# Equim-chan/Mortal

Measured on NVIDIA H100. Metric: table-steps/sec batched self-play, higher is better.
Workload: dtype u8/i32 env + bf16 policy net

## Files before the change

### mortal_b200/csrc/mjx_kernels.cu

```cuda
#include <cstdint>
#include <cstdio>
#include <cstring>
#include <initializer_list>
#include <mutex>
#include <string>
#include <vector>

#include "../../include/mjx.h"
#include "mjx_sp.cuh"
#include "mjx_policy.cuh"
#include "mjx_replay.cuh"
#include "mjx_validate.cuh"
#include "mjx_mjai.cuh"
#include "mjx_mjai_write.cuh"
#include "mjx_stat.cuh"
#include "mjx_grp.cuh"
#include "mjx_reward.cuh"
#include "mjx_invisible.cuh"
#include "mjx_state.cuh"
#include "mjx_nn.cuh"
#include "mjx_tables_host.h"

using namespace mjx;

// ... 424 lines not shown
    recompute_dora_factor(c);

__global__ void k_state_init(TableState* tabs, int n, const u8* player_ids) {
    const int t = blockIdx.x * blockDim.x + threadIdx.x;
    if (t < n) { tabs[t].viewer1 = (u8)(player_ids[t] + 1); tabs[t].gflags = GF_ALIVE; tabs[t].last_kawa_tile = T_NONE;
                 for (int s = 0; s < 4; s++) tabs[t].priv[s].last_self_tsumo = T_NONE; }
}

__global__ void __launch_bounds__(STEP_WARPS * 32) k_state_update(EnvView V, Tables T, const u64* __restrict__ words,
                                                                    const u64* __restrict__ payload, u32* __restrict__ cans) {
    STATE_KERNEL_PROLOGUE
    const u64 w = words[i];
    const int p = c.S->viewer1 - 1;
    if (w != 0) {
        apply_event(c, w, payload ? payload + (size_t)i * REPLAY_KYOKU_WORDS : nullptr, false);
        __syncwarp();
        for (int q = lane; q < NV; q += 32) reinterpret_cast<uint4*>(g)[q] = dst[q];
    }
    if (lane == 0) cans[i] = (u32)c.S->priv[p].cans | ((u32)c.S->priv[p].target_actor << 16);
}

__global__ void __launch_bounds__(STEP_WARPS * 32) k_state_view(EnvView V, Tables T, int index, mjx_player_view* out) {
    STATE_KERNEL_PROLOGUE
    if (i != index) return;
    if (lane == 0) state_view(c, c.S->viewer1 - 1, out);
}

__global__ void __launch_bounds__(STEP_WARPS * 32) k_state_rows(EnvView V, Tables T, const u8* __restrict__ at_kan_select) {
    STATE_KERNEL_PROLOGUE
    const int p = c.S->viewer1 - 1;
    const bool kan = at_kan_select && at_kan_select[i];
    const u16 cans_bits = c.S->priv[p].cans;
    const u64 discards = (cans_bits & CAN_DISCARD) ? discard_candidates(c, p) : 0;
    write_mask_row(c, V, i, legal_mask(c, p, kan, discards));
    if (lane == 0) { V.row_table[i] = i; V.row_seat[i] = (u8)(p | (kan ? 4 : 0)); V.row_step[i] = 0; if (i == 0) *V.n_rows = V.n_tables; }
}

__global__ void __launch_bounds__(STEP_WARPS * 32) k_state_query(EnvView V, Tables T, int index, int what, const i32* __restrict__ args,
                                                                   i32* __restrict__ out) {
    STATE_KERNEL_PROLOGUE
    if (i != index) return;
    const int p = c.S->viewer1 - 1;
    if (what == 0) {
        u8 ura[5];
        const int n_ura = min(max(args[1], 0), 5);
        for (int k = 0; k < n_ura; k++) ura[k] = (u8)args[2 + k];
        bool ok;
        const Point pt = agari_points_ura(c, p, args[0] != 0, ura, n_ura, &ok);
        if (lane == 0) { out[0] = pt.ron; out[1] = pt.tsumo_ko; out[2] = pt.tsumo_oya; out[3] = ok ? 1 : 0; }
    } else if (what == 1) {
        const bool r = rule_based_agari(c, p);
        if (lane == 0) out[0] = r ? 1 : 0;
    } else if (what == 2) {
        const u64 m = discard_candidates(c, p);
        if (lane == 0) { out[0] = (i32)(u32)m; out[1] = (i32)(u32)(m >> 32); }
    } else if (what == 3) {
        EncCtx e; e.S = c.S; e.T = T; e.bm = nullptr; e.sv = nullptr; e.seat = p; e.kan_select = false; e.lane = lane;
        e.dora_factor = c.df; e.parts = 0;
        const u64 m = unconditional_tenpai_discards(e, c);
        if (lane == 0) { out[0] = (i32)(u32)m; out[1] = (i32)(u32)(m >> 32); }
    } else if (what == 4) {
        Reaction r;
        i32 err = 0;
        const bool okd = decode_action(c.S, p, args[0], args[1], r, &err);
        if (lane == 0) {
            u64 w = 0;
            if (okd) {
                const int ty = r.type == R_DAHAI ? LOG_DAHAI : r.type == R_CHI ? LOG_CHI : r.type == R_PON ? LOG_PON :
                               r.type == R_DAIMINKAN ? LOG_DAIMINKAN : r.type == R_KAKAN ? LOG_KAKAN : r.type == R_ANKAN ? LOG_ANKAN :
                               r.type == R_REACH ? LOG_REACH : r.type == R_HORA ? LOG_HORA : r.type == R_RYUKYOKU ? LOG_RYUKYOKU : 0;
                w = log_word(ty, r.actor, r.target, r.pai, r.tsumogiri, 0, r.consumed[0], r.consumed[1], r.consumed[2], r.consumed[3], 0);
            }
            out[0] = (i32)(u32)w; out[1] = (i32)(u32)(w >> 32); out[2] = okd ? 0 : (err ? err : ERR_ILLEGAL_ACTION);
        }
    }
}

constexpr int SP_WARPS = 4;
constexpr int MJX_HOST_COPY_GROUPS = 4;
constexpr int MJX_SP_MAX_LANES = 4;

__global__ void k_sp_begin(SpGlobal G) {
    if (threadIdx.x < SP_SLOTS) G.wl_count[threadIdx.x] = 0;
    if (threadIdx.x == 0) {
        if (G.counters[2]) G.counters[3] += 1;
        G.counters[0] = 0; G.counters[1] = 0; G.counters[2] = 0; G.counters[4] = 0; G.counters[5] = 0;
    }
}

#define SP_ROW_PROLOGUE                                                                         \
    __shared__ u8 s_df[SP_WARPS][40];                                                           \
    const int warp = threadIdx.x >> 5, lane = threadIdx.x & 31;                                 \
    const int gwarp = blockIdx.x * SP_WARPS + warp, nwarps = gridDim.x * SP_WARPS;              \
    SpCtx s; s.G = G; s.T = T; s.df = s_df[warp]; s.lane = lane;

#define SP_ROW_RANGE                                                                            \
    const int span_ = max(min(*V.n_rows, row_hi) - row_lo, 0);                                  \
    const int r0 = row_lo + (int)((long long)span_ * part / parts), r1 = row_lo + (int)((long long)span_ * (part + 1) / parts);

__global__ void __launch_bounds__(SP_WARPS * 32) k_sp_init(SpGlobal G, Tables T, EnvView V, int row_lo, int row_hi, int part, int parts) {
    SP_ROW_PROLOGUE
    SP_ROW_RANGE
    for (int row = r0 + gwarp; row < r1; row += nwarps)
        sp_stage_init(s, V.tables + V.row_table[row], row, V.row_table[row], V.row_seat[row] & 3);
}

template <int KIND>
__global__ void __launch_bounds__(SP_THREADS) k_sp_expand(SpGlobal G, Tables T, int level) {
    __shared__ SpExpandBatch sb;
    SpBlk B; B.tid = threadIdx.x; B.nthr = blockDim.x; B.bid = blockIdx.x; B.nblk = gridDim.x;
    sp_expand_level<KIND>(G, T, sb, B, level);
}

template <int KIND>
__global__ void __launch_bounds__(SP_THREADS) k_sp_eval(SpGlobal G, int level) {
    SpBlk B; B.tid = threadIdx.x; B.nthr = blockDim.x; B.bid = blockIdx.x; B.nblk = gridDim.x;
    if (KIND == 0) {
        __shared__ SpEvalDBatch sd;
        sp_eval_d_level(G, sd, B, level);
    } else {
        __shared__ SpEvalWBatch sw[SP_THREADS / 32];
        sp_eval_w_level<KIND == 2>(G, sw, B, level);
    }
}

__global__ void k_sp_tables(float* p_tab) {
    const int i = blockIdx.x * blockDim.x + threadIdx.x;
    if (i < SP_NTS_DIM * SP_NTS_DIM) sp_fill_ptab_block(p_tab + (size_t)i * 4 * SP_TRI, i / SP_NTS_DIM, i % SP_NTS_DIM);
}

__global__ void k_sp_mark(SpGlobal G, int which) { G.counters[4 + which] = min(G.counters[1], G.edge_cap); }

__global__ void __launch_bounds__(256) k_sp_densify(SpGlobal G) {
    SpBlk B; B.tid = threadIdx.x; B.nthr = blockDim.x; B.bid = blockIdx.x; B.nblk = gridDim.x;
    sp_densify(G, B);
}

__global__ void __launch_bounds__(128) k_sp_score(SpGlobal G, Tables T) {
    const int b = G.counters[4], e_end = G.counters[5];
    for (int e = b + blockIdx.x * blockDim.x + threadIdx.x; e < e_end; e += gridDim.x * blockDim.x) sp_score_edge(G, T, e);
}

__global__ void __launch_bounds__(SP_WARPS * 32) k_sp_finalize(SpGlobal G, Tables T, EnvView V, float* __restrict__ obs, int row_lo,
                                                               int row_hi, int part, int parts) {
    SP_ROW_PROLOGUE
    SP_ROW_RANGE
    for (int row = r0 + gwarp; row < r1; row += nwarps)
        sp_stage_finalize(s, row, obs + (size_t)row * OBS_ROWS_V4 * OBS_COLS);
}

__global__ void __launch_bounds__(256) k_sp_release(SpGlobal G) {
    SpBlk B; B.tid = threadIdx.x; B.nthr = blockDim.x; B.bid = blockIdx.x; B.nblk = gridDim.x;
    sp_release(G, B);
}

__global__ void k_policy_test(EnvView V, int kind, i64* actions, i64* trace, float* q_out) {
    const int n_rows = *V.n_rows;
    for (int r = blockIdx.x * blockDim.x + threadIdx.x; r < n_rows; r += gridDim.x * blockDim.x) {
        const int t = V.row_table[r], seat = V.row_seat[r] & 3, kan = (V.row_seat[r] >> 2) & 1;
        u64 m = 0;
        for (int i = 0; i < ACTION_SPACE; i++) if (V.masks[(size_t)r * ACTION_SPACE + i]) m |= 1ull << i;
        const TableState* S = V.tables + t;
        const SeatPrivate& P = S->priv[seat];
        u64 h = policy_hash(S->nonce, S->key, (u64)t, V.row_step[r], (u32)seat, (u32)kan);
        int a = test_policy(kind, h, kan != 0, m, P.keep_shanten, P.next_shanten);
        actions[r] = a;
// ... 84 lines not shown

template <typename Tp>
int upload(const std::vector<Tp>& v, const Tp** out) {
    Tp* d = nullptr;
    CU(cudaMalloc(&d, v.size() * sizeof(Tp)));
    CU(cudaMemcpy(d, v.data(), v.size() * sizeof(Tp), cudaMemcpyHostToDevice));
    *out = d;
    return 0;
}

}

struct mjx_env {
    int n_tables = 0, row_cap = 0, obs_version = 4, shuffle_kind = 0, quick_eval = 1;
    bool first = true;
    EnvView V;
    u64 *d_nonces = nullptr, *d_keys = nullptr;
    i64* d_dummy_actions = nullptr;
    u8* d_guard = nullptr;
    u8* d_quick_eval = nullptr;
    SpGlobal sp;
    int sp_enabled = 1, sp_wanted = 1;
    SpGlobal sp_lane[MJX_SP_MAX_LANES - 1];
    int sp_lanes = 1, sp_lanes_alloc = 1;
    int sp_grid_x = 10, sp_grid_e = 16;
    int sp_thr_x = SP_THREADS, sp_thr_e = SP_THREADS;
    long long sp_want_slots = 0;
    cudaStream_t sp_stream[MJX_SP_MAX_LANES] = {};
    cudaEvent_t ev_sp_fork = nullptr, ev_sp_store = nullptr, ev_sp_join[MJX_SP_MAX_LANES] = {};
    unsigned char* d_compact = nullptr;
    cudaEvent_t ev_enc[3] = {nullptr, nullptr, nullptr};
    bool time_encode = false;
    ReplayView R{};
    bool replay = false;
    long long r_n_hdr = 0, r_n_kyoku = 0;
    bool viewpoints = false;
    int* d_enc_work = nullptr;
    EncStoreArgs enc_args{};
    cudaStream_t copy_stream = nullptr;
    cudaEvent_t ev_rows = nullptr, ev_sp = nullptr, ev_grp[MJX_HOST_COPY_GROUPS] = {};
    long long launches = 0;
    bool is_state = false;
    u64 *d_state_words = nullptr, *d_state_pay = nullptr;
    u32* d_state_cans = nullptr;
    unsigned char* d_state_misc = nullptr;
};

static void set_enc_args(mjx_env* env, int version) {
    const ObsLayout L = make_layout(version);
    env->enc_args.rows = L.rows; env->enc_args.bm_rows = L.bm_rows; env->enc_args.n_sv = L.n_sv;
    env->enc_args.compact_bytes = L.bm_rows * 8 + L.n_sv * OBS_COLS * 4;
    env->enc_args.n_slices = (L.rows + OBS_SLICE_ROWS - 1) / OBS_SLICE_ROWS;
    env->enc_args.ver = version;
}

template <int VER>
static void launch_features(mjx_env* env, cudaStream_t st) {
    k_encode_features<VER><<<g_sm_count, EncF<VER>::WARPS * 32, EncF<VER>::SMEM, st>>>(env->V, g_T, env->d_compact, env->d_enc_work);
}

static int sp_alloc(SpGlobal& G, long long want) {
    int hc = 1 << 20;
    while (hc < want && hc < (1 << 26)) hc <<= 1;
    G.hash_cap = hc;
    G.p_tab = g_sp_p_tab;
    G.wl_cap = hc / 2;
    G.edge_cap = hc * 2;
    G.score_cap = hc;
    CU(cudaMalloc(&G.hkey, (size_t)G.hash_cap * sizeof(u64)));
    CU(cudaMalloc(&G.nsig, (size_t)G.hash_cap * sizeof(SpSigP)));
    CU(cudaMalloc(&G.einfo, (size_t)G.hash_cap * sizeof(u64)));
    CU(cudaMalloc(&G.vals, (size_t)G.hash_cap * SP_VALS * sizeof(float)));
    CU(cudaMalloc(&G.sid, (size_t)G.hash_cap * sizeof(u32)));
    CU(cudaMalloc(&G.dkey, (size_t)G.hash_cap * sizeof(u64)));
    CU(cudaMalloc(&G.echild, (size_t)G.edge_cap * sizeof(u32)));
    CU(cudaMalloc(&G.evid, (size_t)G.edge_cap * sizeof(u32)));
    CU(cudaMemset(G.evid, 0, (size_t)G.edge_cap * sizeof(u32)));
    CU(cudaMalloc(&G.emeta, (size_t)G.edge_cap * sizeof(u16)));
    CU(cudaMalloc(&G.eowner, (size_t)G.edge_cap * sizeof(u32)));
    CU(cudaMalloc(&G.leaf_scores, (size_t)G.score_cap * 4 * sizeof(float)));
    CU(cudaMalloc(&G.wl, (size_t)SP_SLOTS * G.wl_cap * sizeof(u32)));
    CU(cudaMalloc(&G.wl_count, SP_SLOTS * sizeof(i32)));
    CU(cudaMalloc(&G.counters, 8 * sizeof(i32)));
    CU(cudaMemset(G.counters, 0, 8 * sizeof(i32)));
    CU(cudaMemset(G.wl_count, 0, SP_SLOTS * sizeof(i32)));
    CU(cudaMemset(G.hkey, 0xFF, (size_t)G.hash_cap * sizeof(u64)));
    return MJX_OK;
}
static SpGlobal& sp_of(mjx_env* env, int lane) { return lane == 0 ? env->sp : env->sp_lane[lane - 1]; }
static void sp_free(SpGlobal& G) {
    cudaFree(G.hkey); cudaFree(G.nsig); cudaFree(G.einfo); cudaFree(G.vals); cudaFree(G.sid); cudaFree(G.dkey); cudaFree(G.echild); cudaFree(G.evid); cudaFree(G.emeta);
    cudaFree(G.eowner); cudaFree(G.leaf_scores); cudaFree(G.wl); cudaFree(G.wl_count); cudaFree(G.counters);
}
static int sp_ensure_lanes(mjx_env* env, int lanes) {
    if (!env->ev_sp_fork) {
        CU(cudaEventCreateWithFlags(&env->ev_sp_fork, cudaEventDisableTiming));
        CU(cudaEventCreateWithFlags(&env->ev_sp_store, cudaEventDisableTiming));
    }
    for (int g = 0; g < lanes; g++)
        if (!env->sp_stream[g]) {
            CU(cudaStreamCreateWithFlags(&env->sp_stream[g], cudaStreamNonBlocking));
            CU(cudaEventCreateWithFlags(&env->ev_sp_join[g], cudaEventDisableTiming));
        }
    for (int g = env->sp_lanes_alloc; g < lanes; g++) {
        SpGlobal& G = env->sp_lane[g - 1];
        memset(&G, 0, sizeof G);
        G.rows = env->sp.rows;
        int rc = sp_alloc(G, env->sp_want_slots * 2 / lanes);
        if (rc) return rc;
        env->sp_lanes_alloc = g + 1;
    }
    return MJX_OK;
}

extern "C" {

const char* mjx_last_error(void) { return g_err.c_str(); }

int mjx_init(const char* data_dir, int device) {
    std::lock_guard<std::mutex> lk(g_mu);
    if (g_ready) {
        if (device != g_device) return fail(MJX_ERR_ARG, "mjx_init: already initialised on another device");
        return MJX_OK;
    }
    int n_dev = 0;
    cudaError_t e = cudaGetDeviceCount(&n_dev);
    if (e != cudaSuccess || n_dev == 0)
        return fail(MJX_ERR_CUDA, "mjx_init: no CUDA device (this library has no CPU path)");
    CU(cudaSetDevice(device));
    cudaDeviceProp prop;
    CU(cudaGetDeviceProperties(&prop, device));
    g_sm_count = prop.multiProcessorCount;
    HostTables H;
    if (!load_host_tables(data_dir, H)) return fail(MJX_ERR_TABLES, "mjx_init: " + H.error);
    int rc;
    if ((rc = upload(H.suhai, &g_T.suhai))) return rc;
    if ((rc = upload(H.jihai, &g_T.jihai))) return rc;
    if ((rc = upload(H.agari_keys, &g_T.agari_keys))) return rc;
    if ((rc = upload(H.agari_divs, &g_T.agari_divs))) return rc;
    if ((rc = upload(H.agari_ndivs, &g_T.agari_ndivs))) return rc;
    CU(cudaFuncSetAttribute(k_encode_features<1>, cudaFuncAttributeMaxDynamicSharedMemorySize, (int)EncF<1>::SMEM));
    CU(cudaFuncSetAttribute(k_encode_features<2>, cudaFuncAttributeMaxDynamicSharedMemorySize, (int)EncF<2>::SMEM));
    CU(cudaFuncSetAttribute(k_encode_features<3>, cudaFuncAttributeMaxDynamicSharedMemorySize, (int)EncF<3>::SMEM));
    CU(cudaFuncSetAttribute(k_encode_features<4>, cudaFuncAttributeMaxDynamicSharedMemorySize, (int)EncF<4>::SMEM));
    {
        short tab[4][OBS_MAX_SV];
        for (int v = 1; v <= 4; v++) {
            const ObsLayout L = make_layout(v);
            for (int i = 0; i < OBS_MAX_SV; i++) tab[v - 1][i] = i < L.n_sv ? L.sv_row[i] : (short)-1;
        }
        CU(cudaMemcpyToSymbol(c_sv_row, tab, sizeof tab));
    }
    CU(cudaFuncSetAttribute(k_encode_store, cudaFuncAttributeMaxDynamicSharedMemorySize, (int)ENCS_SMEM_BYTES));
    {
        float* pt = nullptr;
        CU(cudaMalloc(&pt, sizeof(float) * SP_NTS_DIM * SP_NTS_DIM * 4 * SP_TRI));
        k_sp_tables<<<(SP_NTS_DIM * SP_NTS_DIM + 63) / 64, 64>>>(pt);
        CU(cudaGetLastError());
        CU(cudaDeviceSynchronize());
        g_sp_p_tab = pt;
    }
    g_device = device;
    g_ready = true;
    return MJX_OK;
}

int mjx_obs_rows(int version) {
    switch (version) {
        case 1: return 938;
        case 2: return 942;
        case 3: return 934;
        case 4: return 1012;
        default: return MJX_ERR_ARG;
    }
}
// ... 1134 lines not shown
```

### mortal_b200/csrc/mjx_sp.cuh

```cuda
#pragma once
#include "mjx_obs.cuh"

namespace mjx {

constexpr int SP_T_MAX = 17;
constexpr int SP_SHANTEN_THRES = 3;
constexpr int SP_MAX_TILES_LEFT = 34 * 4 - 1 - 13;
constexpr int SP_SLOTS = 8;
constexpr int SP_B = 32;
constexpr int SP_THREADS = 128;
constexpr int SP_MAX_EDGES = 37;
constexpr u64 SP_EMPTY = ~0ull;
constexpr u32 SP_NO_CHILD = 0xFFFFFFFFu;
constexpr u32 SP_DR_NONE = 0x3FFFFu, SP_DI_NONE = 0xFFFFFFu;
constexpr int SP_VALS = 3 * SP_T_MAX;

#ifdef MJX_HOST_EMUL
#define SP_FMUL(a, b) ((a) * (b))
#define SP_FADD(a, b) ((a) + (b))
#define SP_FDIV(a, b) ((a) / (b))
#define SP_SYNC() ((void)0)
#else
#define SP_FMUL(a, b) __fmul_rn((a), (b))
#define SP_FADD(a, b) __fadd_rn((a), (b))
// ... 48 lines not shown
MJX_HD u32 sp_hash64(u64 x) {
    x ^= x >> 33; x *= 0xff51afd7ed558ccdull; x ^= x >> 33; x *= 0xc4ceb9fe1a85ec53ull; x ^= x >> 33;
    return (u32)x;
}

struct alignas(16) SpSigP { u32 w[4]; };
MJX_D SpSigP sp_sig_pack(const HandSig& h) {
    SpSigP p;
    p.w[0] = h.idx[0] | ((u32)h.kinds << 21); p.w[1] = h.idx[1] | ((u32)h.pairs << 21);
    p.w[2] = h.idx[2] | ((u32)h.kkinds << 21); p.w[3] = h.idx[3] | ((u32)h.kpairs << 21);
    return p;
}
MJX_D HandSig sp_sig_unpack(const SpSigP& p) {
    HandSig h;
    for (int i = 0; i < 4; i++) h.idx[i] = p.w[i] & 0x1FFFFFu;
    h.kinds = (int)(p.w[0] >> 21); h.pairs = (int)(p.w[1] >> 21); h.kkinds = (int)(p.w[2] >> 21); h.kpairs = (int)(p.w[3] >> 21);
    return h;
}

template <bool ADD>
MJX_D int sp_candidate_shanten(const Tables& T, const SpSigP& sg, const u8* others, int t, int c0, int len_div3) {
    const int sx = t / 9, pos = t - 9 * sx;
    const u32 w5 = sx < 3 ? c_pow5[pos] : c_pow5[pos + 2];
    const u32 idx = (sg.w[sx] & 0x1FFFFFu) + (ADD ? w5 : 0u - w5);
    const u64 r = sx < 3 ? ld_row(T.suhai, idx, SUHAI_ROWS) : ld_row(T.jihai, idx, JIHAI_ROWS);
    int v = 1 << 20;
#pragma unroll
    for (int a = 0; a <= 4; a++) {
        if (a <= len_div3) {
            const int b = len_div3 - a;
            v = min(v, (int)others[5 + a] + (int)((r >> (4 * b)) & 0xF));
            v = min(v, (int)others[a] + (int)((r >> (4 * (5 + b))) & 0xF));
        }
    }
    int sh = v - 1;
    if (sh <= 0 || len_div3 < 4) return sh;
    int kinds = (int)(sg.w[0] >> 21), pairs = (int)(sg.w[1] >> 21), kkinds = (int)(sg.w[2] >> 21), kpairs = (int)(sg.w[3] >> 21);
    const bool yao = is_yaokyuu(t);
    if (ADD) { kinds += c0 == 0; pairs += c0 == 1; if (yao) { kkinds += c0 == 0; kpairs += c0 == 1; } }
    else { kinds -= c0 == 1; pairs -= c0 == 2; if (yao) { kkinds -= c0 == 1; kpairs -= c0 == 2; } }
    sh = min(sh, 7 - pairs + max(7 - kinds, 0) - 1);
    if (sh > 0) sh = min(sh, 14 - kkinds - (kpairs > 0 ? 1 : 0) - 1);
    return sh;
}

struct SpRow {
    u8 tehai_len_div3, is_menzen, prefer_riichi, calc_double_riichi, calc_haitei;
    u8 bakaze, jikaze, num_doras_in_fuuro, n_dora;
    u8 dora_ind[5];
    u8 melds[16];
    u8 n_chis, n_pons, n_minkans, n_ankans;
    u8 T;
    u8 n_left;
    u8 avail;
    u8 has_values;
    u8 can_discard;
    u8 cd_flag;
    u8 after_riichi, last_self_tsumo;
    i8 cur_shanten;
    u8 seat;
    i32 table;
    u32 root;
    float fallback_ev;
    SpKey root_key;
};

struct SpGlobal {
    SpRow* rows;
    u64* hkey;
    SpSigP* nsig;
    u64* einfo;
    u64* dkey;
    float* vals;
    u32* sid;
    u32* echild;
    u32* evid;
    u16* emeta;
    u32* eowner;
    float* leaf_scores;
    u32* wl;
    i32* wl_count;
    const float* p_tab;
    i32* counters;
    i32 row_base;
    i32 hash_cap, wl_cap, edge_cap, score_cap;
};

MJX_CONST float c_uradora_prob[5][13] = {
    {0.639485f, 0.327801f, 0.0327134f, 0.f, 0.f, 0.f, 0.f, 0.f, 0.f, 0.f, 0.f, 0.f, 0.f},
    {0.406736f, 0.42281f, 0.147966f, 0.021674f, 0.0008142f, 0.f, 0.f, 0.f, 0.f, 0.f, 0.f, 0.f, 0.f},
    {0.257516f, 0.406819f, 0.246851f, 0.0757724f, 0.0122266f, 0.0008004f, 1.43e-5f, 0.f, 0.f, 0.f, 0.f, 0.f, 0.f},
    {0.162199f, 0.346513f, 0.301539f, 0.142396f, 0.0401276f, 0.0066491f, 0.0005575f, 1.85e-5f, 0.f, 0.f, 0.f, 0.f, 0.f},
    {0.101768f, 0.275319f, 0.313742f, 0.20189f, 0.081774f, 0.0215394f, 0.0035918f, 0.0003607f, 1.52e-5f, 3e-7f, 0.f, 0.f, 0.f},
};
MJX_CONST u8 c_discard_priority[38] = {6, 5, 4, 3, 2, 3, 4, 5, 6, 6, 5, 4, 3, 2, 3, 4, 5, 6, 6, 5, 4, 3, 2, 3, 4, 5, 6,
                                        7, 7, 7, 7, 7, 7, 7, 1, 1, 1, 0};

MJX_D int cmp_discard_priority(int l, int r) {
    int pl = c_discard_priority[l], pr = c_discard_priority[r];
    if (pl != pr) return pl < pr ? -1 : 1;
    if (l != r) return r < l ? -1 : 1;
    return 0;
}

struct SpBlk { int tid, nthr, bid, nblk; };

MJX_HD bool sp_slot_is_w(int slot) { return (slot & 1) != 0; }
MJX_HD int sp_slot_shanten(int slot) { return 3 - (slot >> 1); }
MJX_D float* sp_vals(const SpGlobal& G, u32 vid, int which) { return G.vals + ((size_t)vid * 3 + which) * SP_T_MAX; }
MJX_D u32 sp_einfo_begin(u64 e) { return (u32)e; }
MJX_D int sp_einfo_n(u64 e) { return (int)((e >> 32) & 0xFF); }
MJX_D int sp_einfo_sum(u64 e) { return (int)((e >> 40) & 0xFF); }
MJX_D int sp_einfo_cmask(u64 e) { return (int)((e >> 48) & 0xF); }

MJX_D void sp_set_overflow(const SpGlobal& G) { G.counters[2] = 1; }

constexpr u32 SP_SID_POS = (1u << 28) - 1u;
MJX_D u32 sp_level_base(const SpGlobal& G, int level) {
    u32 b = 0;
    for (int l = 0; l < level; l++) b += (u32)min(G.wl_count[l], G.wl_cap);
    return b;
}
MJX_D u32 sp_vid(const SpGlobal& G, u32 slot) {
    const u32 s = G.sid[slot];
    return sp_level_base(G, (int)(s >> 28)) + (s & SP_SID_POS);
}
MJX_DN void sp_densify(const SpGlobal& G, const SpBlk& B) {
    if (G.counters[2]) return;
    u32 base[SP_SLOTS];
    for (int l = 0; l < SP_SLOTS; l++) base[l] = sp_level_base(G, l);
    const int n = min(G.counters[1], G.edge_cap), leaf_b = G.counters[4], leaf_e = G.counters[5];
    for (int e = B.bid * B.nthr + B.tid; e < n; e += B.nblk * B.nthr) {
        if (e >= leaf_b && e < leaf_e) continue;
        const u32 c = G.echild[e];
        u32 v = SP_NO_CHILD;
        if (c != SP_NO_CHILD) { const u32 sd = G.sid[c]; v = base[sd >> 28] + (sd & SP_SID_POS); }
        G.evid[e] = v;
    }
}

MJX_D void sp_prefetch(const float* p) {
#ifndef MJX_HOST_EMUL
    asm volatile("prefetch.global.L1 [%0];" ::"l"(p));
    asm volatile("prefetch.global.L1 [%0];" ::"l"(p + 32));
#else
    (void)p;
#endif
}
MJX_D i32 sp_atomic_add(i32* p, i32 v) {
#ifdef MJX_HOST_EMUL
    const i32 o = *p; *p += v; return o;
#else
    return atomicAdd(p, v);
#endif
}
MJX_D void sp_atomic_or(u32* p, u32 v) {
#ifdef MJX_HOST_EMUL
    *p |= v;
#else
    atomicOr(p, v);
#endif
}

MJX_DN u32 sp_intern(const SpGlobal& G, u64 key, bool& won) {
    const u32 mask = (u32)G.hash_cap - 1;
    u32 h = sp_hash64(key) & mask;
    won = false;
    for (int probe = 0; probe < 8192; probe++, h = (h + 1) & mask) {
#ifdef MJX_HOST_EMUL
        const u64 cur = G.hkey[h];
        if (cur == key) return h;
        if (cur == SP_EMPTY) { G.hkey[h] = key; won = true; return h; }
#else
        const u64 cur = __ldcg(reinterpret_cast<const unsigned long long*>(G.hkey + h));
        if (cur == key) return h;
        if (cur == SP_EMPTY) {
            const u64 prev = atomicCAS(reinterpret_cast<unsigned long long*>(G.hkey + h), (unsigned long long)SP_EMPTY,
                                       (unsigned long long)key);
            if (prev == SP_EMPTY) { won = true; return h; }
            if (prev == key) return h;
        }
#endif
    }
    sp_set_overflow(G);
    return SP_NO_CHILD;
}

struct SpExpandBatch {
    u64 key[SP_B];
    u32 slot[SP_B];
    SpSigP sig[SP_B];
    u8 akas[SP_B], len[SP_B];
    u8 teh[SP_B][34], wall[SP_B][34];
    u8 oth[SP_B][4][12];
    u32 cand[SP_B][2], eff[SP_B][2];
    u8 split[SP_B], ne[SP_B], sumreq[SP_B], cmask[SP_B];
    u16 cand_off[SP_B + 1], e_off[SP_B + 1];
    u16 cand_list[SP_B * 34];
    u32 edge[SP_B * SP_MAX_EDGES];
    u32 win[SP_B * SP_MAX_EDGES];
    i32 n_cand, n_edge, e_base, n_win, w_base;
};

MJX_D u64 sp_mask64(const u32* m) { return (u64)m[0] | ((u64)m[1] << 32); }

template <int KIND>
MJX_DN void sp_expand_batch(const SpGlobal& G, const Tables& T, SpExpandBatch& S, const SpBlk& B, int level, int first, int nb) {
    constexpr bool IS_W = KIND != 0, LEAF = KIND == 2;
    const int k = sp_slot_shanten(level);
    const u32* list = G.wl + (size_t)level * G.wl_cap;
    SP_PFOR(st, nb) {
        const u32 slot = list[first + st];
        const u64 key = G.hkey[slot];
        const SpRow& R = G.rows[sp_key_row(key)];
        S.slot[st] = slot; S.key[st] = key;
        S.sig[st] = G.nsig[slot];
        S.akas[st] = (u8)sp_key_akas(R.root_key.akas, sp_key_dr(key), sp_key_di(key));
        S.len[st] = R.tehai_len_div3;
        S.cand[st][0] = S.cand[st][1] = S.eff[st][0] = S.eff[st][1] = 0;
    }
    if (B.tid == 0) S.n_win = 0;
    SP_SYNC();
    SP_PFOR(it, nb * 34) {
        const int st = it / 34, t = it - st * 34;
        const SpRow& R = G.rows[sp_key_row(S.key[st])];
        S.teh[st][t] = R.root_key.tehai[t]; S.wall[st][t] = R.root_key.wall[t];
    }
    SP_PFOR(it, nb * 4) {
        const int st = it >> 2, sx = it & 3;
        const HandSig h = sp_sig_unpack(S.sig[st]);
        Row10 acc;
        bool first = true;
        for (int q = 0; q < 4; q++) {
            if (q == sx) continue;
            const Row10 r = unpack_row(q < 3 ? ld_row(T.suhai, h.idx[q], SUHAI_ROWS) : ld_row(T.jihai, h.idx[q], JIHAI_ROWS));
            if (first) { acc = r; first = false; } else add_suhai_full(acc, r);
        }
        for (int q = 0; q < 10; q++) S.oth[st][sx][q] = (u8)acc.v[q];
    }
    SP_SYNC();
    SP_PFOR(st, nb) {
        const u64 key = S.key[st];
        const u32 dr = sp_key_dr(key), di = sp_key_di(key);
        for (int i = 0; i < 3; i++) { const int f = (int)((dr >> (6 * i)) & 63u); if (f != 63) { S.teh[st][deaka(f)] += 1; S.wall[st][deaka(f)] -= 1; } }
        for (int i = 0; i < 4; i++) { const int f = (int)((di >> (6 * i)) & 63u); if (f != 63) S.teh[st][deaka(f)] -= 1; }
        u64 m = 0;
        for (int t = 0; t < 34; t++) if ((IS_W ? S.wall[st][t] : S.teh[st][t]) > 0) m |= 1ull << t;
        S.cand[st][0] = (u32)m; S.cand[st][1] = (u32)(m >> 32);
    }
    SP_SYNC();
    if (B.tid == 0) {
        int acc = 0;
        for (int st = 0; st < nb; st++) { S.cand_off[st] = (u16)acc; acc += mjx_popcll(sp_mask64(S.cand[st])); }
        S.cand_off[nb] = (u16)acc; S.n_cand = acc;
    }
    SP_SYNC();
    SP_PFOR(it, nb * 34) {
        const int st = it / 34, t = it - st * 34;
        const u64 m = sp_mask64(S.cand[st]);
        if ((m >> t) & 1) S.cand_list[S.cand_off[st] + mjx_popcll(m & ((1ull << t) - 1))] = (u16)((st << 6) | t);
    }
    SP_SYNC();
    SP_PFOR(i, S.n_cand) {
        const int st = S.cand_list[i] >> 6, t = S.cand_list[i] & 63;
        const int sh = sp_candidate_shanten<IS_W>(T, S.sig[st], S.oth[st][t / 9], t, S.teh[st][t], S.len[st]);
        const bool ok = IS_W ? sh - k == -1 : sh == k;
        if (ok) sp_atomic_or(&S.eff[st][t >> 5], 1u << (t & 31));
    }
    SP_SYNC();
    SP_PFOR(st, nb) {
        const u64 eff = sp_mask64(S.eff[st]);
        int split = 0, sum = 0, cmask = 0;
        if (IS_W) {
            for (int s5 = 0; s5 < 3; s5++) {
                const int t5 = 4 + 9 * s5;
                if (((eff >> t5) & 1) && ((S.akas[st] >> (3 + s5)) & 1) && S.wall[st][t5] >= 2) split |= 1 << s5;
            }
            for (u64 rest = eff; rest; rest &= rest - 1) {
                const int t = mjx_ffsll(rest) - 1, cnt = S.wall[st][t];
                sum += cnt;
                const int s5 = (t == T_5M || t == T_5P || t == T_5S) ? t / 9 : -1;
                if (s5 >= 0 && ((S.akas[st] >> (3 + s5)) & 1)) { cmask |= 1; if (cnt >= 2) cmask |= 1 << (cnt - 2); }
                else cmask |= 1 << (cnt - 1);
            }
        }
        S.split[st] = (u8)split;
        S.cmask[st] = (u8)cmask;
        S.ne[st] = (u8)(mjx_popcll(eff) + mjx_popc((u32)split));
        S.sumreq[st] = (u8)sum;
    }
    SP_SYNC();
    if (B.tid == 0) {
        int acc = 0;
        for (int st = 0; st < nb; st++) { S.e_off[st] = (u16)acc; acc += S.ne[st]; }
        S.e_off[nb] = (u16)acc;
        int eb = sp_atomic_add(&G.counters[1], acc);
        if (eb + acc > G.edge_cap) { sp_set_overflow(G); acc = 0; eb = 0; }
        S.n_edge = acc; S.e_base = eb;
    }
    SP_SYNC();
    SP_PFOR(st, nb) {
        const int ne = S.n_edge ? S.ne[st] : 0;
        const u32 vid = sp_level_base(G, level) + (u32)(first + st);
        G.einfo[vid] = (u64)(u32)(S.e_base + S.e_off[st]) | ((u64)ne << 32) | ((u64)S.sumreq[st] << 40) | ((u64)S.cmask[st] << 48);
        G.dkey[vid] = S.key[st];
    }
    if (S.n_edge) SP_PFOR(it, nb * 34) {
        const int st = it / 34, t = it - st * 34;
        const u64 eff = sp_mask64(S.eff[st]);
        if (!((eff >> t) & 1)) continue;
        int off = S.e_off[st] + mjx_popcll(eff & ((1ull << t) - 1));
        for (int s5 = 0; s5 < 3; s5++) off += ((S.split[st] >> s5) & 1) && 4 + 9 * s5 < t;
        const int suit5 = (t == T_5M || t == T_5P || t == T_5S) ? t / 9 : -1;
        if (IS_W) {
            const int count = S.wall[st][t];
            if (suit5 >= 0 && ((S.akas[st] >> (3 + suit5)) & 1)) {
                if (count >= 2) { S.edge[off] = (u32)st | ((u32)t << 8) | ((u32)(count - 1) << 16); off++; }
                S.edge[off] = (u32)st | ((u32)(T_5MR + suit5) << 8) | (1u << 16);
            } else {
                S.edge[off] = (u32)st | ((u32)t << 8) | ((u32)count << 16);
            }
        } else {
            int tile = t;
            if (suit5 >= 0 && ((S.akas[st] >> suit5) & 1) && S.teh[st][t] == 1) tile = T_5MR + suit5;
            S.edge[off] = (u32)st | ((u32)tile << 8);
        }
    }
    SP_SYNC();
    SP_PFOR(e, S.n_edge) {
        const u32 d = S.edge[e];
        const int st = (int)(d & 0xFF), tile = (int)((d >> 8) & 0xFF), cnt = (int)(d >> 16);
        const int ge = S.e_base + e;
        G.emeta[ge] = (u16)(tile | (cnt << 6));
        if (LEAF) { G.eowner[ge] = sp_level_base(G, level) + (u32)(first + st); continue; }
        const u64 key = S.key[st];
        const int t = deaka(tile);
        const u64 ckey = IS_W ? sp_key_make(sp_key_row(key), sp_tuple_insert(sp_key_dr(key), 3, (u32)tile), sp_key_di(key))
                              : sp_key_make(sp_key_row(key), sp_key_dr(key), sp_tuple_insert(sp_key_di(key), 4, (u32)tile));
        bool won;
        const u32 child = sp_intern(G, ckey, won);
        G.echild[ge] = child;
        if (won) {
            G.nsig[child] = sp_sig_pack(sig_variant(sp_sig_unpack(S.sig[st]), t, IS_W ? +1 : -1, S.teh[st][t]));
            S.win[sp_atomic_add(&S.n_win, 1)] = child;
        }
    }
    SP_SYNC();
    if (!LEAF) {
        if (B.tid == 0) {
            int wb = sp_atomic_add(&G.wl_count[level + 1], S.n_win);
            if (wb + S.n_win > G.wl_cap) { sp_set_overflow(G); S.n_win = 0; wb = 0; }
            S.w_base = wb;
        }
        SP_SYNC();
        u32* next = G.wl + (size_t)(level + 1) * G.wl_cap;
        SP_PFOR(i, S.n_win) {
            next[S.w_base + i] = S.win[i];
            G.sid[S.win[i]] = ((u32)(level + 1) << 28) | (u32)(S.w_base + i);
        }
        SP_SYNC();
    }
}

template <int KIND>
MJX_DN void sp_expand_level(const SpGlobal& G, const Tables& T, SpExpandBatch& S, const SpBlk& B, int level) {
    const int n = min(G.wl_count[level], G.wl_cap);
    for (int first = B.bid * SP_B; first < n; first += B.nblk * SP_B) sp_expand_batch<KIND>(G, T, S, B, level, first, min(SP_B, n - first));
}

MJX_DN bool sp_get_score(const Tables& T, const SpRow& P, const u8* tehai13, const u8* wall_in, int akas, int win_tile, float* scores) {
    u8 th[34];
    for (int i = 0; i < 34; i++) th[i] = tehai13[i];
    const int wid = deaka(win_tile);
    th[wid] += 1;
    const int akas_in_hand = (akas & 7) | (is_aka(win_tile) ? (1 << (win_tile - T_5MR)) : 0);
    u8 wall[34];
    for (int i = 0; i < 34; i++) wall[i] = wall_in[i];
    wall[wid] -= 1;
    AgariQuery q;
    q.tehai = th;
    q.chis = P.melds; q.pons = P.melds + 4; q.minkans = P.melds + 8; q.ankans = P.melds + 12;
    q.n_chis = P.n_chis; q.n_pons = P.n_pons; q.n_minkans = P.n_minkans; q.n_ankans = P.n_ankans;
    q.bakaze = P.bakaze; q.jikaze = P.jikaze; q.winning_tile = wid; q.is_ron = false; q.is_menzen = P.is_menzen != 0;
    const bool is_oya = P.jikaze == T_E;
    const int additional = P.is_menzen ? (P.prefer_riichi ? 2 : 1) : 0;
    int doras = mjx_popc((u32)akas_in_hand) + P.num_doras_in_fuuro;
    for (int i = 0; i < P.n_dora; i++) doras += th[tile_next(P.dora_ind[i])];
    Agari a = agari_with(T, q, additional, doras & 0xFF);
    if (a.kind == 0) return false;
    if (a.kind == 2) {
        float v = (float)tsumo_total(point_yakuman(is_oya, a.yakuman), is_oya);
        for (int i = 0; i < 4; i++) scores[i] = v;
        return true;
    }
    const int fu = a.fu, han = a.han;
    const bool assume_riichi = P.is_menzen && P.prefer_riichi;
    const int n_extra = !assume_riichi ? 4 : (P.n_dora == 1 ? 8 : 16);
    float pts[16];
    for (int h = 0; h < n_extra; h++) { bool ok; pts[h] = (float)tsumo_total(point_calc(is_oya, fu, han + h, &ok), is_oya); }
    for (int i = 0; i < 4; i++) scores[i] = 0.f;
    if (assume_riichi && P.n_dora == 1) {
        int n_ind[5] = {0, 0, 0, 0, 0};
        int sum_ind = 0, n_left = 0;
        for (int t = 0; t < 34; t++) n_left += wall[t];
        for (int t = 0; t < 34; t++) {
            int cnt = th[t];
            if (cnt == 0) continue;
            int ic = wall[tile_prev(t)];
            n_ind[cnt] = (n_ind[cnt] + ic) & 0xFF;
            sum_ind = (sum_ind + ic) & 0xFF;
        }
        float up[5];
        up[0] = SP_FDIV((float)((n_left - sum_ind) & 0xFF), (float)n_left);
        for (int i = 1; i < 5; i++) up[i] = SP_FDIV((float)n_ind[i], (float)n_left);
        for (int i = 0; i < 4; i++)
            for (int j = 0; j < 5; j++) {
                if (up[j] == 0.f) continue;
                scores[i] = SP_FADD(scores[i], SP_FMUL(pts[i + j], up[j]));
            }
    } else if (assume_riichi && P.n_dora > 1) {
        for (int i = 0; i < 4; i++)
            for (int j = 0; j < 13; j++) {
                float p = c_uradora_prob[P.n_dora - 1][j];
                if (p == 0.f) continue;
                scores[i] = SP_FADD(scores[i], SP_FMUL(pts[i + j], p));
            }
    } else {
        for (int i = 0; i < 4; i++) scores[i] = pts[i];
    }
    return true;
}

MJX_DN void sp_score_edge(const SpGlobal& G, const Tables& T, int e) {
    const u32 node = G.eowner[e];
    const u64 key = G.dkey[node];
    const SpRow& P = G.rows[sp_key_row(key)];
    const u32 dr = sp_key_dr(key), di = sp_key_di(key);
    u8 th[34], wall[34];
    for (int t = 0; t < 34; t++) { th[t] = P.root_key.tehai[t]; wall[t] = P.root_key.wall[t]; }
    for (int i = 0; i < 3; i++) { const int f = (int)((dr >> (6 * i)) & 63u); if (f != 63) { th[deaka(f)] += 1; wall[deaka(f)] -= 1; } }
    for (int i = 0; i < 4; i++) { const int f = (int)((di >> (6 * i)) & 63u); if (f != 63) th[deaka(f)] -= 1; }
    float sc[4];
    const u16 m = G.emeta[e];
    const bool ok = sp_get_score(T, P, th, wall, sp_key_akas(P.root_key.akas, dr, di), m & 63, sc);
    const int le = e - G.counters[4];
    if (le >= G.score_cap) G.counters[2] = 1;
    if (!ok) G.emeta[e] = (u16)(m | 0x8000);
    else if (le >= 0 && le < G.score_cap) {
        float* o = G.leaf_scores + (size_t)le * 4;
        o[0] = sc[0]; o[1] = sc[1]; o[2] = sc[2]; o[3] = sc[3];
    }
}

struct SpEvalDBatch {
    u32 vid[SP_B], ebeg[SP_B];
    u8 ne[SP_B], T[SP_B], d[SP_B];
    u16 off[SP_B + 1];
    i32 n_items;
};
constexpr int SP_NTS_DIM = SP_MAX_TILES_LEFT + 2;
constexpr int SP_TRI = SP_T_MAX * (SP_T_MAX + 1) / 2;
MJX_HD int sp_tri_row(int i) { return SP_T_MAX * i - i * (i - 1) / 2; }
MJX_D size_t sp_ptab_index(int n_left, int i0) { return ((size_t)n_left * SP_NTS_DIM + (size_t)i0) * 4 * SP_TRI; }
MJX_D void sp_fill_ptab_block(float* blk, int n_left, int i0) {
    float nts[SP_T_MAX];
    float v = 1.f;
    for (int j = 0; j < SP_T_MAX; j++) {
        const bool ok = i0 <= n_left && j <= n_left - i0;
        nts[j] = ok ? v : 0.f;
        if (ok && j < n_left - i0) v = SP_FDIV(SP_FMUL(v, (float)(n_left - i0 - j)), (float)(n_left - j));
    }
    for (int c = 0; c < 4; c++)
        for (int j = 0; j < SP_T_MAX; j++) {
            const float tpj = (n_left - j > 0 && nts[j] != 0.f) ? SP_FMUL(SP_FDIV((float)(c + 1), (float)(n_left - j)), nts[j]) : 0.f;
            for (int i = 0; i <= j; i++) blk[c * SP_TRI + sp_tri_row(i) + (j - i)] = nts[i] != 0.f ? SP_FDIV(tpj, nts[i]) : 0.f;
        }
}

constexpr int SP_WB = 7;
struct SpEvalWBatch {
    u32 vid[SP_WB], ebeg[SP_WB], pbase[SP_WB];
    u8 ne[SP_WB], T[SP_WB], d[SP_WB], flags[SP_WB], jend[SP_WB];
    u16 aoff[SP_WB + 1];
    i32 n_a;
};
#ifdef MJX_HOST_EMUL
#define SP_WSYNC() ((void)0)
#else
#define SP_WSYNC() __syncwarp()
#endif
template <typename Tb>
MJX_D int sp_find_state(const u16* off, int nb, int item) {
    int lo = 0, hi = nb - 1;
    while (lo < hi) {
        const int mid = (lo + hi + 1) >> 1;
        if ((int)off[mid] <= item) lo = mid; else hi = mid - 1;
    }
    return lo;
}

template <bool LEAF>
MJX_DN void sp_eval_w_batch(const SpGlobal& G, SpEvalWBatch& S, const SpBlk& B, int level, int first, int nb) {
    const int k = LEAF ? 0 : sp_slot_shanten(level);
    const u32 vbase = sp_level_base(G, level) + (u32)first;
    SP_PFOR(st, nb) {
        const u64 key = G.dkey[vbase + st];
        const SpRow& R = G.rows[sp_key_row(key)];
        const u64 ei = G.einfo[vbase + st];
        const int Tn = R.T, n_left = R.n_left, i0 = sp_einfo_sum(ei);
        const bool row_ok = i0 <= n_left && i0 <= SP_MAX_TILES_LEFT;
        const int lim = row_ok ? min(Tn - 1, n_left - i0) : -1;
        S.vid[st] = vbase + (u32)st; S.ebeg[st] = sp_einfo_begin(ei); S.ne[st] = (u8)sp_einfo_n(ei);
        S.T[st] = (u8)Tn; S.d[st] = (u8)min(sp_key_depth(key), Tn);
#ifdef MJX_HOST_EMUL
        for (int i = 0; i < S.d[st]; i++) { float* o = G.vals + (size_t)S.vid[st] * SP_VALS; o[i] = o[SP_T_MAX + i] = o[2 * SP_T_MAX + i] = __builtin_nanf(""); }
#endif
        const bool ar = R.is_menzen && R.prefer_riichi;
        S.flags[st] = (u8)((ar ? 1 : 0) | (R.calc_double_riichi ? 2 : 0) | (R.calc_haitei ? 4 : 0));
        S.jend[st] = (u8)max(0, min(Tn, lim + 1));
        S.pbase[st] = row_ok ? (u32)sp_ptab_index(n_left, i0) : 0u;
    }
    SP_WSYNC();
    if (B.tid == 0) {
        int aa = 0;
        for (int st = 0; st < nb; st++) { S.aoff[st] = (u16)aa; aa += (S.T[st] - S.d[st] + 1) / 2; }
        S.aoff[nb] = (u16)aa; S.n_a = aa;
    }
    SP_WSYNC();
    SP_PFOR(item, S.n_a) {
        const int st = sp_find_state<int>(S.aoff, nb, item), p = item - S.aoff[st];
        const int Tn = S.T[st], ne = S.ne[st], jend = S.jend[st];
        const u32 eb = S.ebeg[st];
        const float* Pb = G.p_tab + S.pbase[st];
        const bool assume_riichi = (S.flags[st] & 1) != 0, dbl = (S.flags[st] & 2) != 0, haitei = (S.flags[st] & 4) != 0;
        const int i0 = S.d[st] + p, i1 = Tn - 1 - p;
        const bool two = i1 > i0;
        float t0 = 0.f, w0 = 0.f, v0 = 0.f, t1 = 0.f, w1 = 0.f, v1 = 0.f;
        u16 meta_n = ne ? G.emeta[eb] : (u16)0;
        u32 child_n = (!LEAF && ne) ? G.evid[eb] : 0u;
        for (int e = 0; e < ne; e++) {
            const u16 meta = meta_n;
            const u32 child = child_n;
            if (e + 1 < ne) { meta_n = G.emeta[eb + e + 1]; if (!LEAF) child_n = G.evid[eb + e + 1]; }
            if (!LEAF && e + 1 < ne && child_n != SP_NO_CHILD) sp_prefetch(G.vals + (size_t)child_n * SP_VALS);
            const float* Pc = Pb + (((meta >> 6) & 7) - 1) * SP_TRI;
            const float* P0 = Pc + sp_tri_row(i0) - i0;
            const float* P1 = Pc + sp_tri_row(i1 > 0 ? i1 : 0) - i1;
            float s0 = 0.f, s1 = 0.f, s2 = 0.f, s3 = 0.f;
            const float* cv = nullptr;
            if (LEAF) {
                if (meta & 0x8000) continue;
                const int le = (int)(eb + e) - G.counters[4];
                if (le < 0 || le >= G.score_cap) continue;
                const float* sc = G.leaf_scores + (size_t)le * 4;
                s0 = sc[0]; s1 = sc[1]; s2 = sc[2]; s3 = sc[3];
            } else {
                if (child == SP_NO_CHILD) continue;
                cv = G.vals + (size_t)child * SP_VALS;
            }
            if (i0 < jend)
                for (int j = i0; j < jend; j++) {
                    const float prob = P0[j];
                    if (LEAF) {
                        const int han_plus = (assume_riichi && dbl && i0 == 0) + (assume_riichi && j == i0) + (haitei && j == Tn - 1);
                        const float sv = han_plus == 0 ? s0 : (han_plus == 1 ? s1 : (han_plus == 2 ? s2 : s3));
                        w0 = SP_FADD(w0, prob);
                        v0 = SP_FADD(v0, SP_FMUL(prob, sv));
                    } else {
                        if (k == 1) t0 = SP_FADD(t0, prob);
                        if (j < Tn - 1) {
                            if (k > 1) t0 = SP_FADD(t0, SP_FMUL(prob, cv[j + 1]));
                            w0 = SP_FADD(w0, SP_FMUL(prob, cv[SP_T_MAX + j + 1]));
                            v0 = SP_FADD(v0, SP_FMUL(prob, cv[2 * SP_T_MAX + j + 1]));
                        }
                    }
                }
            if (two && i1 < jend)
                for (int j = i1; j < jend; j++) {
                    const float prob = P1[j];
                    if (LEAF) {
                        const int han_plus = (assume_riichi && j == i1) + (haitei && j == Tn - 1);
                        const float sv = han_plus == 0 ? s0 : (han_plus == 1 ? s1 : s2);
                        w1 = SP_FADD(w1, prob);
                        v1 = SP_FADD(v1, SP_FMUL(prob, sv));
                    } else {
                        if (k == 1) t1 = SP_FADD(t1, prob);
                        if (j < Tn - 1) {
                            if (k > 1) t1 = SP_FADD(t1, SP_FMUL(prob, cv[j + 1]));
                            w1 = SP_FADD(w1, SP_FMUL(prob, cv[SP_T_MAX + j + 1]));
                            v1 = SP_FADD(v1, SP_FMUL(prob, cv[2 * SP_T_MAX + j + 1]));
                        }
                    }
                }
        }
        float* o = G.vals + (size_t)S.vid[st] * SP_VALS;
        o[i0] = t0; o[SP_T_MAX + i0] = w0; o[2 * SP_T_MAX + i0] = v0;
        if (two) { o[i1] = t1; o[SP_T_MAX + i1] = w1; o[2 * SP_T_MAX + i1] = v1; }
    }
    SP_WSYNC();
}

MJX_DN void sp_eval_d_batch(const SpGlobal& G, SpEvalDBatch& S, const SpBlk& B, int level, int first, int nb) {
    const u32 vbase = sp_level_base(G, level) + (u32)first;
    SP_PFOR(st, nb) {
        const u64 ei = G.einfo[vbase + st];
        S.vid[st] = vbase + (u32)st; S.ebeg[st] = sp_einfo_begin(ei); S.ne[st] = (u8)sp_einfo_n(ei);
        const u64 key = G.dkey[vbase + st];
        S.T[st] = G.rows[sp_key_row(key)].T; S.d[st] = (u8)min(sp_key_depth(key), (int)S.T[st]);
#ifdef MJX_HOST_EMUL
        for (int i = 0; i < S.d[st]; i++) { float* o = G.vals + (size_t)S.vid[st] * SP_VALS; o[i] = o[SP_T_MAX + i] = o[2 * SP_T_MAX + i] = __builtin_nanf(""); }
#endif
    }
    SP_SYNC();
    if (B.tid == 0) {
        int acc = 0;
        for (int st = 0; st < nb; st++) { S.off[st] = (u16)acc; acc += S.T[st] - S.d[st]; }
        S.off[nb] = (u16)acc; S.n_items = acc;
    }
    SP_SYNC();
    SP_PFOR(item, S.n_items) {
        const int st = sp_find_state<int>(S.off, nb, item), i = S.d[st] + item - S.off[st];
        const int ne = S.ne[st];
        const u32 eb = S.ebeg[st];
        const float FMIN = -3.40282347e+38f;
        float bt = FMIN, bw = FMIN, bv = FMIN;
        int best_tile = T_UNK;
        i32 best_value = (i32)0x80000000;
        u32 child_n = ne ? G.evid[eb] : SP_NO_CHILD;
        for (int e = 0; e < ne; e++) {
            const u32 child = child_n;
            if (e + 1 < ne) { child_n = G.evid[eb + e + 1]; if (child_n != SP_NO_CHILD && i == S.d[st]) sp_prefetch(G.vals + (size_t)child_n * SP_VALS); }
            if (child == SP_NO_CHILD) continue;
            const int tile = G.emeta[eb + e] & 63;
            const float* cv = G.vals + (size_t)child * SP_VALS;
            const float v = cv[2 * SP_T_MAX + i];
            const i32 value = (i32)v;
            if (value > best_value || (value == best_value && cmp_discard_priority(tile, best_tile) > 0)) {
                bt = cv[i]; bw = cv[SP_T_MAX + i]; bv = v;
                best_value = value; best_tile = tile;
            }
        }
        float* o = G.vals + (size_t)S.vid[st] * SP_VALS;
        o[i] = bt; o[SP_T_MAX + i] = bw; o[2 * SP_T_MAX + i] = bv;
    }
    SP_SYNC();
}

MJX_DN void sp_eval_d_level(const SpGlobal& G, SpEvalDBatch& S, const SpBlk& B, int level) {
    if (G.counters[2]) return;
    const int n = min(G.wl_count[level], G.wl_cap);
    for (int first = B.bid * SP_B; first < n; first += B.nblk * SP_B) sp_eval_d_batch(G, S, B, level, first, min(SP_B, n - first));
}
template <bool LEAF>
MJX_DN void sp_eval_w_level(const SpGlobal& G, SpEvalWBatch* S, const SpBlk& B, int level) {
    if (G.counters[2]) return;
    const int n = min(G.wl_count[level], G.wl_cap);
    const int lanes = B.nthr >= 32 ? 32 : B.nthr, wpc = B.nthr / lanes, warp = B.tid / lanes;
    SpBlk W; W.tid = B.tid - warp * lanes; W.nthr = lanes; W.bid = B.bid * wpc + warp; W.nblk = B.nblk * wpc;
    for (int first = W.bid * SP_WB; first < n; first += W.nblk * SP_WB)
        sp_eval_w_batch<LEAF>(G, S[warp], W, level, first, min(SP_WB, n - first));
}

MJX_DN void sp_release(const SpGlobal& G, const SpBlk& B) {
    const int gtid = B.bid * B.nthr + B.tid, gn = B.nblk * B.nthr;
    if (G.counters[2]) {
        for (int i = gtid; i < G.hash_cap; i += gn) G.hkey[i] = SP_EMPTY;
        return;
    }
    for (int level = 0; level < SP_SLOTS; level++) {
        const int n = min(G.wl_count[level], G.wl_cap);
        const u32* list = G.wl + (size_t)level * G.wl_cap;
        for (int i = gtid; i < n; i += gn) G.hkey[list[i]] = SP_EMPTY;
    }
}

struct SpCtx {
    SpGlobal G;
    Tables T;
    u8* df;
    int lane;
};

struct SpCand {
    int tile;
    int node;
    u32 vid;
    u64 required;
    int num_required;
    bool shanten_down;
    float t0, w0, e0;
};

MJX_D float clamp01(float v) { return fminf(fmaxf(v, 0.f), 1.f); }
MJX_D int cmp_f32(float a, float b) { return a < b ? -1 : (a > b ? 1 : 0); }

MJX_D int sp_cand_cmp(const SpCand& l, const SpCand& r, int by , bool has_values) {
    if (l.tile == r.tile) return 0;
    if (by == 0 && has_values) {
        int o = cmp_f32(l.e0, r.e0); if (o) return o;
        o = cmp_f32(l.w0, r.w0); if (o) return o;
        o = cmp_f32(l.t0, r.t0); if (o) return o;
    }
    if (!l.shanten_down && r.shanten_down) return 1;
    if (l.shanten_down && !r.shanten_down) return -1;
    if (l.num_required != r.num_required) return l.num_required < r.num_required ? -1 : 1;
    return cmp_discard_priority(l.tile, r.tile);
}

MJX_DN void sp_required(const SpCtx& s, const Ctx& c, int len, const u8* tehai, const u8* wall, u64* set, int* num) {
    const HandSig base = hand_sig(tehai);
    const int cur = shanten_all_sig(s.T, base, len);
    u64 req, unused;
    tile_eval2(c, true, [&](int t) {
        if (wall[t] == 0) return 0;
        return shanten_all_sig(s.T, sig_variant(base, t, +1, tehai[t]), len) < cur ? 1 : 0;
    }, req, unused);
    int n = 0;
    for (u64 rest = req; rest; rest &= rest - 1) n += wall[mjx_ffsll(rest) - 1];
    *set = req;
    *num = n & 0xFF;
}

MJX_D int real_time_shanten(const Tables& T, const TableState* S, int p) {
    const SeatPrivate& P = S->priv[p];
    if (!(P.cans & CAN_DISCARD)) return P.shanten;
    if (P.shanten > 0) return (P.flags & PF_HAS_NEXT_SHANTEN_DISCARD) ? P.shanten - 1 : P.shanten;
    if (P.last_self_tsumo != T_NONE) return ((P.waits >> deaka(P.last_self_tsumo)) & 1) ? -1 : 0;
    return shanten_all(T, P.tehai, P.tehai_len_div3);
}

MJX_DN void sp_stage_init(SpCtx& s, const TableState* S, int row, int table, int seat) {
    const int p = seat;
    const SeatPrivate& PV = S->priv[p];
    const SeatPublic& PU = S->pub[p];
    const u16 cans = PV.cans;
    MJX_FOR_TILES(s, t) {
        int f = 0;
        for (int q = 0; q < S->n_dora; q++) f += tile_next(S->wall[60 - q]) == t;
        s.df[t] = (u8)f;
    }
    MJX_END_TILES(s);
    const u8* df = s.df;
    Ctx c;
// ... 345 lines not shown
```

Measured before the change: 241,900.

## Use atomic work counters for dynamic batch distribution in search levels

Replaces the static strided assignment of 32-item (or 7-item per warp) batches in the expand, d-eval and w-eval level loops with dynamic claiming through per-level atomic counters held in a new device array. The counters are reset in k_sp_begin. The aim is to balance uneven per-batch cost across blocks and warps, so fast workers stop idling while others finish long batches. In exchange it adds one global atomic plus a block or warp sync per claimed batch. It also risks a shared-variable race when a worker exits the loop without a trailing sync.

After: 243,400, median of 6. Within noise of the previous version (+0.6%).

```diff
diff --git a/mortal_b200/csrc/mjx_kernels.cu b/mortal_b200/csrc/mjx_kernels.cu
--- a/mortal_b200/csrc/mjx_kernels.cu
+++ b/mortal_b200/csrc/mjx_kernels.cu
@@ -530,6 +530,7 @@
 
 __global__ void k_sp_begin(SpGlobal G) {
     if (threadIdx.x < SP_SLOTS) G.wl_count[threadIdx.x] = 0;
+    if (threadIdx.x < SP_WORK) G.work[threadIdx.x] = 0;
     if (threadIdx.x == 0) {
         if (G.counters[2]) G.counters[3] += 1;
         G.counters[0] = 0; G.counters[1] = 0; G.counters[2] = 0; G.counters[4] = 0; G.counters[5] = 0;
@@ -780,6 +781,7 @@
     CU(cudaMalloc(&G.wl, (size_t)SP_SLOTS * G.wl_cap * sizeof(u32)));
     CU(cudaMalloc(&G.wl_count, SP_SLOTS * sizeof(i32)));
     CU(cudaMalloc(&G.counters, 8 * sizeof(i32)));
+    CU(cudaMalloc(&G.work, SP_WORK * sizeof(i32)));
     CU(cudaMemset(G.counters, 0, 8 * sizeof(i32)));
     CU(cudaMemset(G.wl_count, 0, SP_SLOTS * sizeof(i32)));
     CU(cudaMemset(G.hkey, 0xFF, (size_t)G.hash_cap * sizeof(u64)));
@@ -788,7 +790,7 @@
 static SpGlobal& sp_of(mjx_env* env, int lane) { return lane == 0 ? env->sp : env->sp_lane[lane - 1]; }
 static void sp_free(SpGlobal& G) {
     cudaFree(G.hkey); cudaFree(G.nsig); cudaFree(G.einfo); cudaFree(G.vals); cudaFree(G.sid); cudaFree(G.dkey); cudaFree(G.echild); cudaFree(G.evid); cudaFree(G.emeta);
-    cudaFree(G.eowner); cudaFree(G.leaf_scores); cudaFree(G.wl); cudaFree(G.wl_count); cudaFree(G.counters);
+    cudaFree(G.eowner); cudaFree(G.leaf_scores); cudaFree(G.wl); cudaFree(G.wl_count); cudaFree(G.counters); cudaFree(G.work);
 }
 static int sp_ensure_lanes(mjx_env* env, int lanes) {
     if (!env->ev_sp_fork) {
diff --git a/mortal_b200/csrc/mjx_sp.cuh b/mortal_b200/csrc/mjx_sp.cuh
--- a/mortal_b200/csrc/mjx_sp.cuh
+++ b/mortal_b200/csrc/mjx_sp.cuh
@@ -154,6 +154,7 @@
     i32* wl_count;
     const float* p_tab;
     i32* counters;
+    i32* work;
     i32 row_base;
     i32 hash_cap, wl_cap, edge_cap, score_cap;
 };
@@ -176,6 +177,7 @@
 }
 
 struct SpBlk { int tid, nthr, bid, nblk; };
+constexpr int SP_WORK = 2 * SP_SLOTS;
 
 MJX_HD bool sp_slot_is_w(int slot) { return (slot & 1) != 0; }
 MJX_HD int sp_slot_shanten(int slot) { return 3 - (slot >> 1); }
@@ -272,6 +274,7 @@
     u32 edge[SP_B * SP_MAX_EDGES];
     u32 win[SP_B * SP_MAX_EDGES];
     i32 n_cand, n_edge, e_base, n_win, w_base;
+    i32 next;
 };
 
 MJX_D u64 sp_mask64(const u32* m) { return (u64)m[0] | ((u64)m[1] << 32); }
@@ -437,7 +440,17 @@
 template <int KIND>
 MJX_DN void sp_expand_level(const SpGlobal& G, const Tables& T, SpExpandBatch& S, const SpBlk& B, int level) {
     const int n = min(G.wl_count[level], G.wl_cap);
+#ifdef MJX_HOST_EMUL
     for (int first = B.bid * SP_B; first < n; first += B.nblk * SP_B) sp_expand_batch<KIND>(G, T, S, B, level, first, min(SP_B, n - first));
+#else
+    for (;;) {
+        if (B.tid == 0) S.next = atomicAdd(&G.work[level], 1) * SP_B;
+        SP_SYNC();
+        const int first = S.next;
+        if (first >= n) break;
+        sp_expand_batch<KIND>(G, T, S, B, level, first, min(SP_B, n - first));
+    }
+#endif
 }
 
 MJX_DN bool sp_get_score(const Tables& T, const SpRow& P, const u8* tehai13, const u8* wall_in, int akas, int win_tile, float* scores) {
@@ -529,6 +542,7 @@
     u8 ne[SP_B], T[SP_B], d[SP_B];
     u16 off[SP_B + 1];
     i32 n_items;
+    i32 next;
 };
 constexpr int SP_NTS_DIM = SP_MAX_TILES_LEFT + 2;
 constexpr int SP_TRI = SP_T_MAX * (SP_T_MAX + 1) / 2;
@@ -555,6 +569,7 @@
     u8 ne[SP_WB], T[SP_WB], d[SP_WB], flags[SP_WB], jend[SP_WB];
     u16 aoff[SP_WB + 1];
     i32 n_a;
+    i32 next;
 };
 #ifdef MJX_HOST_EMUL
 #define SP_WSYNC() ((void)0)
@@ -721,7 +736,17 @@
 MJX_DN void sp_eval_d_level(const SpGlobal& G, SpEvalDBatch& S, const SpBlk& B, int level) {
     if (G.counters[2]) return;
     const int n = min(G.wl_count[level], G.wl_cap);
+#ifdef MJX_HOST_EMUL
     for (int first = B.bid * SP_B; first < n; first += B.nblk * SP_B) sp_eval_d_batch(G, S, B, level, first, min(SP_B, n - first));
+#else
+    for (;;) {
+        if (B.tid == 0) S.next = atomicAdd(&G.work[SP_SLOTS + level], 1) * SP_B;
+        SP_SYNC();
+        const int first = S.next;
+        if (first >= n) break;
+        sp_eval_d_batch(G, S, B, level, first, min(SP_B, n - first));
+    }
+#endif
 }
 template <bool LEAF>
 MJX_DN void sp_eval_w_level(const SpGlobal& G, SpEvalWBatch* S, const SpBlk& B, int level) {
@@ -729,8 +754,18 @@
     const int n = min(G.wl_count[level], G.wl_cap);
     const int lanes = B.nthr >= 32 ? 32 : B.nthr, wpc = B.nthr / lanes, warp = B.tid / lanes;
     SpBlk W; W.tid = B.tid - warp * lanes; W.nthr = lanes; W.bid = B.bid * wpc + warp; W.nblk = B.nblk * wpc;
+#ifdef MJX_HOST_EMUL
     for (int first = W.bid * SP_WB; first < n; first += W.nblk * SP_WB)
         sp_eval_w_batch<LEAF>(G, S[warp], W, level, first, min(SP_WB, n - first));
+#else
+    for (;;) {
+        if (W.tid == 0) S[warp].next = atomicAdd(&G.work[SP_SLOTS + level], 1) * SP_WB;
+        SP_WSYNC();
+        const int first = S[warp].next;
+        if (first >= n) break;
+        sp_eval_w_batch<LEAF>(G, S[warp], W, level, first, min(SP_WB, n - first));
+    }
+#endif
 }
 
 MJX_DN void sp_release(const SpGlobal& G, const SpBlk& B) {
```
